# yinwoods/k8s-scheduler

Measured on AMD Instinct MI355X. Metric: pod-node evaluations/sec, higher is better.
Workload: dtype f64

## Files before the change

k8s-scheduler_amd/csrc/ksched_pipe.hip:

```cpp
#include <hip/hip_fp16.h>
#include <hip/hip_runtime.h>

#include <cstdio>
#include <cstdlib>

#include "ksched_commit.h"
#include "ksched_merge.h"

#ifndef KSCHED_PIPE_PART
#define KSCHED_PIPE_PART 0
#endif

namespace ksched {

namespace {

constexpr int kSW = kPipeScoreWaves;
constexpr int kMT = kPipeMergeThreads;
constexpr int kMW = kMT / 64;
constexpr int kMS = kPipeMergeSlots;
constexpr int kPU = 4;
#ifndef KSCHED_XCHG_DEBUG
#define KSCHED_XCHG_DEBUG 0
#endif
constexpr int kSPU = 4;
constexpr int kPairCap = 48;
constexpr int kPairMax = 1024;

__device__ __forceinline__ int bperm(int v, int src) { return __builtin_amdgcn_ds_bpermute(src << 2, v); }
__device__ __forceinline__ int64_t bperm64(int64_t v, int src) {
    const uint32_t lo = (uint32_t)bperm((int)(uint32_t)(uint64_t)v, src);
    const uint32_t hi = (uint32_t)bperm((int)(uint32_t)((uint64_t)v >> 32), src);
    return (int64_t)(((uint64_t)hi << 32) | lo);
}
__device__ __forceinline__ int wave_incl_sum(int v) {
    const int lane = (int)__lane_id();
#pragma unroll
    for (int d = 1; d < 64; d <<= 1) {
        const int t = bperm(v, lane >= d ? lane - d : 0);
        v += lane >= d ? t : 0;
    }
    return v;
}

__device__ __forceinline__ void role_sync(unsigned *ctr, unsigned &target, unsigned nwaves) {
    __builtin_amdgcn_fence(__ATOMIC_RELEASE, "workgroup");
    target += nwaves;
    if ((threadIdx.x & 63) == 0) __hip_atomic_fetch_add(ctr, 1u, __ATOMIC_RELAXED, __HIP_MEMORY_SCOPE_WORKGROUP);
    while (__hip_atomic_load(ctr, __ATOMIC_RELAXED, __HIP_MEMORY_SCOPE_WORKGROUP) < target) __builtin_amdgcn_s_sleep(1);
    __builtin_amdgcn_fence(__ATOMIC_ACQUIRE, "workgroup");
}

struct alignas(16) PipeCtl {
    unsigned sbar, mbar;
    int32_t s_stop, m_stop;
    int64_t s_p0, s_done;
    int64_t m_p0, m_done;
    int32_t c_stop;
    int32_t s_ex;
    int32_t s_scr;
    int32_t s_pairs;
    int32_t n_ok, n_err;
    int64_t n_p0, n_done;
};
constexpr size_t kPipeCtlBytes = 128;
static_assert(sizeof(PipeCtl) <= kPipeCtlBytes, "PipeCtl");

__device__ __forceinline__ bool spin_ge(const PersistArgs &P, int slot, const unsigned long long *p,
                                        unsigned long long v, unsigned long long *seen) {
    return poll_ge(p, v, P.timeout_ticks, &P.ctl->polls_rmw, seen, P.prog ? P.prog + kProgWords * slot + 2 : nullptr);
}

__device__ __forceinline__ void set_err(int32_t *err, int32_t code) { atomicCAS(err, 0, code); }

__device__ __forceinline__ void st_sys(uint64_t *p, uint64_t v) {
    __hip_atomic_store(p, v, __ATOMIC_RELAXED, __HIP_MEMORY_SCOPE_SYSTEM);
}
__device__ __forceinline__ uint64_t ld_sys(const uint64_t *p) {
    return __hip_atomic_load(p, __ATOMIC_RELAXED, __HIP_MEMORY_SCOPE_SYSTEM);
}
__device__ __forceinline__ bool granule_wait(const uint64_t *p, uint32_t tag, int64_t limit, uint32_t *word) {
    const uint32_t t16 = gran_tag(tag);
    if (!gran_dec(ld_sys(p), t16, word)) {
        const uint64_t t0 = wall_clock64();
        do {
            if ((int64_t)(wall_clock64() - t0) > limit) return false;
            __builtin_amdgcn_s_sleep(1);
        } while (!gran_dec(ld_sys(p), t16, word));
    }
    return true;
}

template <int K>
__device__ __forceinline__ void rank_merge_msgs(const uint32_t *all, int R, Rec *out, int64_t *out_fc) {
    constexpr int MW = msg_words(K);
    const int lane = threadIdx.x & 63;
    const bool has = lane < R;
    const uint32_t *msg = all + (has ? lane : 0) * MW;
    auto rec_key = [&](int q) {
        return __longlong_as_double((long long)(((uint64_t)msg[q * kRecWords + 1] << 32) | msg[q * kRecWords]));
    };
    int n = 0;
    if (has) {
#pragma unroll
        for (int q = 0; q < K; ++q) n += msg[q * kRecWords + 3] != 0;
    }
    const bool cut = has && msg[13] != 0;
    int64_t cnt = has ? (int64_t)(((uint64_t)msg[K * kRecWords + 1] << 32) | msg[K * kRecWords]) : 0;
    cnt = wave_sum_i64(cnt);
    double ck = (cut && n > 0) ? rec_key(n - 1) : -__builtin_inf();
    int32_t ci = (cut && n > 0) ? (int32_t)msg[(n - 1) * kRecWords + 2] : kNoIdx;
    const bool anycut = __ballot(cut) != 0;
    {
        int32_t aux = 0;
        wave_argbest(ck, ci, aux);
    }
    int h = 0;
    double mk = -__builtin_inf();
    int32_t mi = kNoIdx, msrc = -1;
    for (int r = 0; r < K; ++r) {
        double k = (h < n) ? rec_key(h) : -__builtin_inf();
        int32_t ix = (h < n) ? (int32_t)msg[h * kRecWords + 2] : kNoIdx;
        int32_t src = lane * K + h;
        wave_argbest(k, ix, src);
        if (ix == kNoIdx) break;
        if (src == lane * K + h) ++h;
        if (lane == r) { mk = k; mi = ix; msrc = src; }
// ... 52 lines not shown
#pragma unroll
        for (int j = i; j >= 1; --j) {
            const uint32_t a = t[j - 1], c = t[j];
            t[j - 1] = a > c ? a : c;
            t[j] = a > c ? c : a;
        }
    }
}

template <int KC>
__device__ __forceinline__ void topk_merge_u32(uint32_t (&t)[KC], const uint32_t (&u)[KC]) {
    uint32_t v[KC];
#pragma unroll
    for (int q = 0; q < KC; ++q) v[q] = t[q] > u[KC - 1 - q] ? t[q] : u[KC - 1 - q];
#pragma unroll
    for (int d = KC / 2; d >= 1; d >>= 1) {
#pragma unroll
        for (int i = 0; i < KC; ++i) {
            if ((i & d) == 0) {
                const uint32_t a = v[i], b = v[i + d];
                v[i] = a > b ? a : b;
                v[i + d] = a > b ? b : a;
            }
        }
    }
#pragma unroll
    for (int q = 0; q < KC; ++q) t[q] = v[q];
}

template <int S, int KC>
__device__ __forceinline__ void fold_stage(double (&k)[KC], int32_t (&ix)[KC]) {
    double ok[KC];
    int32_t oi[KC];
#pragma unroll
    for (int q = 0; q < KC; ++q) {
        ok[q] = wpartner_f64<S>(k[q]);
        oi[q] = (int32_t)wpartner<S>((uint32_t)ix[q]);
    }
    double vk[KC];
    int32_t vi[KC];
#pragma unroll
    for (int q = 0; q < KC; ++q) {
        const bool t = better(ok[KC - 1 - q], oi[KC - 1 - q], k[q], ix[q]);
        vk[q] = t ? ok[KC - 1 - q] : k[q];
        vi[q] = t ? oi[KC - 1 - q] : ix[q];
    }
#pragma unroll
    for (int d = KC / 2; d >= 1; d >>= 1) {
#pragma unroll
        for (int i = 0; i < KC; ++i) {
            if ((i & d) == 0) {
                const bool t = better(vk[i + d], vi[i + d], vk[i], vi[i]);
                const double a = vk[i], bb = vk[i + d];
                const int32_t ai = vi[i], bi = vi[i + d];
                vk[i] = t ? bb : a; vi[i] = t ? bi : ai;
                vk[i + d] = t ? a : bb; vi[i + d] = t ? ai : bi;
            }
        }
    }
#pragma unroll
    for (int q = 0; q < KC; ++q) { k[q] = vk[q]; ix[q] = vi[q]; }
}

template <int KC, int K>
struct ScoreLayout {
    static constexpr size_t fold_list_bytes = (size_t)kSW * KC * 64 * 12 + 64 * 4;
    __host__ __device__ static size_t fold_bytes(int R) {
        const size_t scr = (size_t)kSW * KC * 64 * 4 + kSW * 4 + (size_t)2 * kSW * ((R + kSW - 1) / kSW) * 2;
        return scr > fold_list_bytes ? scr : fold_list_bytes;
    }
    __host__ __device__ static size_t rows_off() { return kPipeCtlBytes; }
    __host__ __device__ static size_t fold_off(int R) { return kPipeCtlBytes + (size_t)R * sizeof(NodeRec); }
    __host__ __device__ static size_t total(int R) { return fold_off(R) + (fold_bytes(R) + 15) / 16 * 16; }
    __host__ __device__ static size_t ysq_off(int R) { return total(R); }
    __host__ __device__ static size_t total_screen(int R) { return total(R) + (size_t)R * 16; }
    __host__ __device__ static size_t hrec_off(int R) { return total_screen(R); }
    __host__ __device__ static int hrec_qw(int R) { return ((R + kSW - 1) / kSW + 1) / 2 * 2; }
    __host__ __device__ static size_t hrec_bytes(int R) { return (size_t)kSW * hrec_qw(R) * 64 * 2; }
    __host__ __device__ static size_t total_with_hrec(int R) { return total_screen(R) + hrec_bytes(R); }
    __host__ __device__ static size_t pair_off(int R) {
        const size_t QW = (size_t)(R + kSW - 1) / kSW;
        return ((size_t)kSW * KC * 64 * 4 + kSW * 4 + 4 * kSW * QW + 15) / 16 * 16;
    }
    static constexpr size_t pair_bytes = 64 * 4 * 2 + (size_t)kPairMax * 8 + (size_t)64 * kPairCap * 2;
    __host__ __device__ static bool pairs_fit(int R) { return pair_off(R) + pair_bytes <= (size_t)kSW * KC * 64 * 12; }
};
struct PairArea {
    uint32_t *cnt;
    uint32_t *nel;
    double *key;
    uint16_t *row;
};

struct alignas(16) MergeCtl {
    unsigned mbar;
    int32_t m_stop;
    int64_t m_p0, m_done;
    int32_t m_w, pad;
    unsigned long long m_q;
};
template <int KC, int K>
struct MergeLayout {
    static constexpr size_t ctl_bytes = 64;
    static constexpr size_t merge_bytes = (sizeof(MergeSmem<KC, K, kMT>) + 15) / 16 * 16;
    static constexpr size_t msg_bytes = ((size_t)(1 + kMaxXchgRanks) * msg_words(K) * 4 + 15) / 16 * 16;
    static constexpr size_t slot_bytes = ctl_bytes + merge_bytes + msg_bytes;
    static constexpr size_t total = kMS * slot_bytes;
};
static_assert(sizeof(MergeCtl) <= 64, "MergeCtl");

constexpr size_t kCanaryBytes = 128;
constexpr size_t commit_loc_bytes() { return (sizeof(PersistLocal) + 15) / 16 * 16 + kCanaryBytes; }
template <int K>
constexpr size_t commit_total_bytes() { return commit_loc_bytes() + spc_lds_bytes<K, kPipeThreads, true>(); }
static_assert(commit_total_bytes<16>() <= 160 * 1024, "the persistent commit's LDS (lag-3 slots)");
static_assert(commit_loc_bytes() + spc_small_bytes<16, kPipeThreads, true>() + 256 <= 65536,
              "the persistent commit's arrays in front of S reach LDS immediate offsets");

template <int KC, int K, int PRIO, int DOM, bool LAB, bool F53>
__device__ __forceinline__ void score_role(const PersistArgs &P, char *smem, const int g) {
    PipeCtl *pc = reinterpret_cast<PipeCtl *>(smem);
    const int R = P.rows_per_wg;
    NodeRec *rows = reinterpret_cast<NodeRec *>(smem + ScoreLayout<KC, K>::rows_off());
    char *fold = smem + ScoreLayout<KC, K>::fold_off(R);
    float4 *ysq = reinterpret_cast<float4 *>(smem + ScoreLayout<KC, K>::ysq_off(R));
    uint16_t *hrec = reinterpret_cast<uint16_t *>(smem + ScoreLayout<KC, K>::hrec_off(R));
    int32_t *s_cnt = reinterpret_cast<int32_t *>(fold + (size_t)kSW * KC * 64 * 12);
    PairArea pr;
    {
        char *pa = fold + ScoreLayout<KC, K>::pair_off(R);
        pr.cnt = reinterpret_cast<uint32_t *>(pa);
        pr.nel = pr.cnt + 64;
        pr.key = reinterpret_cast<double *>(pa + 512);
        pr.row = reinterpret_cast<uint16_t *>(pa + 512 + (size_t)kPairMax * 8);
    }
    constexpr int kST = kSW * 64;
    const int tid = threadIdx.x;
    const int lane = tid & 63;
    const int wave = __builtin_amdgcn_readfirstlane(tid >> 6);
    const int G = P.G;
    const int64_t n = P.n_local, NP = P.pods.p;
    Ctl *ctl = P.ctl;
    auto sync = [&]() { __syncthreads(); };
    for (int e = tid; e < R * 6; e += kST) {
        const int r = e / 6, piece = e % 6;
        const int64_t j = g + (int64_t)r * G;
        if (j < n) reinterpret_cast<int4 *>(rows + r)[piece] = reinterpret_cast<const int4 *>(P.nodes + j)[piece];
    }
    if (tid == 0) pc->n_ok = 0;
    sync();
    if (P.screen_ok) {
        for (int r = tid; r < R; r += kST) {
            const NodeRec &nd = rows[r];
            ysq[r] = make_float4(screen_recip(nd.a[0]), screen_recip(nd.a[1]), screen_recip(nd.a[2]), 0.0f);
        }
    }
    const double y3 = recip(3.0);
    constexpr bool kScreen = PRIO == kPrioResource && F53;
    constexpr bool kPairs = kScreen;
    const bool pairs_ok = kPairs && !P.no_pairs && ScoreLayout<KC, K>::pairs_fit(R);
    constexpr int kScreenOffBatches = 16;
    constexpr bool kPrefetch = kSW > 8;
    int64_t scr_off_until = 0;
    int64_t ex_rows = 0, scan_rows = 0;
    const int64_t Rvalid = (n - g + G - 1) / G;
    int64_t nact = 0;
    int idle = 0;
    unsigned long long early_c = 0;
    unsigned long long pre_c = 0;
    auto load_apply = [&](int64_t bb, int stop, int64_t *p0v, int64_t *donev, int *errv) {
        int nxv = 0;
        u32x4 x0 = {0u, 0u, 0u, 0u}, x1 = {0u, 0u, 0u, 0u}, x2 = {0u, 0u, 0u, 0u};
        const XBuf *xb =
            reinterpret_cast<const XBuf *>(P.xring + (size_t)((bb >= kPipeLag ? bb - kPipeLag : 0) % 4) * P.xbuf_bytes);
        if (lane == 0) {
            *p0v = (int64_t)ld_coh(&ctl->plan[bb % kPlanRing]);
            *donev = bb >= kPipeLag ? (int64_t)ld_coh(&ctl->cursor_at[(bb - kPipeLag) % kPlanRing]) : 0;
            *errv = __hip_atomic_load(P.err, __ATOMIC_RELAXED, __HIP_MEMORY_SCOPE_AGENT);
        }
        if (bb >= kPipeLag && !stop) {
            const uint64_t hdr = ld_coh(&xb->count);
            nxv = (uint32_t)(hdr >> 32) == (uint32_t)(bb - kPipeLag) ? (int)(uint32_t)hdr : 0;
            if (lane < 2 * P.B) {
                const __amdgpu_buffer_rsrc_t rs = coh_rsrc(xb->e);
                const uint32_t o = (uint32_t)lane * kXRecPipe;
                x0 = ld_coh16(rs, o); x1 = ld_coh16(rs, o + 16); x2 = ld_coh16(rs, o + 32);
            }
        }
        auto apply = [&](const u32x4 &c0, const u32x4 &c1, const u32x4 &c2) {
            const int64_t j = (int64_t)(int32_t)c0.y - P.node_offset;
            if (j < 0 || j >= n || j % G != g) return;
            const int64_t a0 = w64(c0.z, c0.w), a1 = w64(c1.y, c1.z), a2 = w64(c1.w, c2.y);
            set_row(rows + j / G, a0, a1, a2);
            if (P.screen_ok) ysq[j / G] = make_float4(screen_recip(a0), screen_recip(a1), screen_recip(a2), 0.0f);
            st_coh(&P.nodes[j].a[0], (uint64_t)a0);
            st_coh(&P.nodes[j].a[1], (uint64_t)a1);
            st_coh(&P.nodes[j].a[2], (uint64_t)a2);
        };
        if (lane < nxv) apply(x0, x1, x2);
        for (int e = 64 + lane; e < nxv; e += 64) {
            const __amdgpu_buffer_rsrc_t rs = coh_rsrc(xb->e);
            const uint32_t o = (uint32_t)e * kXRecPipe;
            apply(ld_coh16(rs, o), ld_coh16(rs, o + 16), ld_coh16(rs, o + 32));
        }
    };
    for (int64_t b = 0;; ++b) {
        if (wave == 0) {
            if (kPrefetch && __builtin_amdgcn_readfirstlane(pc->n_ok)) {
                if (lane == 0) {
                    pc->s_p0 = pc->n_p0;
                    pc->s_done = pc->n_done;
                    pc->s_stop = pc->n_err != 0 ? 3 : 0;
                    pc->s_scr = kScreen && P.screen_ok && !P.no_screen && b >= scr_off_until;
                    pc->s_ex = 0;
                    pc->n_ok = 0;
                }
            } else {
                int stop = 0;
                jitter_at(P.jitter, b, 1);
                if (lane == 0) {
                    unsigned long long seen = 0;
                    const unsigned long long need = (unsigned long long)(b - kPipeLag + 1);
                    if (b >= kPipeLag && early_c < need) {
                        prog_at(P, g, b, kProgWaitCommit, 0);
                        if (!spin_ge(P, g, &ctl->committed_x[g % kCtlReplicas].v, need, &seen)) {
                            set_err(P.err, kErrWaitCommit);
                            prog_at(P, g, b, kProgWaitCommit | kProgTimedOut, seen);
                            stop = 2;
                        }
                    }
                    if (g == 0) trace_at(P, b, 6);
                }
                stop = __builtin_amdgcn_readfirstlane(stop);
                int64_t p0v = 0, donev = 0;
                int errv = 0;
                load_apply(b, stop, &p0v, &donev, &errv);
                if (lane == 0) {
                    pc->s_p0 = p0v;
                    pc->s_done = donev;
                    pc->s_stop = errv != 0 ? 3 : stop;
                    pc->s_scr = kScreen && P.screen_ok && !P.no_screen && b >= scr_off_until;
                    pc->s_ex = 0;
                }
            }
        }
        sync();
        if (kPrefetch && wave == kSW - 1) asm volatile("s_waitcnt vmcnt(0)" ::: "memory");
        if (pc->s_stop) return;
        const int64_t p0 = pc->s_p0;
        if (pc->s_done >= NP) break;
        if (p0 < 0 || p0 >= NP) {
            if (tid == 0) prog_at(P, g, b, kProgIdle, (uint64_t)p0);
            if (++idle > kPlanRing) {
                if (tid == 0) set_err(P.err, kErrScorePlan);
                return;
            }
            sync();
            continue;
        }
        idle = 0;
        ++nact;
        if (tid == 0) {
            if (g == 0) trace_at(P, b, 0);
            prog_at(P, g, b, kProgScan, 0);
        }
        const uint64_t t_go = ((P.trace || P.trace_wg) && tid == 0) ? wall_clock64() : 0;
        if (tid < 64) s_cnt[tid] = 0;
        if (kPairs && tid < 64) { pr.cnt[tid] = 0; pr.nel[tid] = 0; }
        bool pairs = false;
        int pT = 0, pincl = 0, pexcl = 0;
        const int64_t pod = p0 + lane;
        const bool active = (lane < P.B) && (pod < NP);
        const int64_t rc = active ? P.pods.rc[pod] : 0;
        const int64_t rm = active ? P.pods.rm[pod] : 0;
        const int64_t rp = active ? P.pods.rp[pod] : 0;
        const uint64_t sel = (LAB && active) ? P.pods.sel[pod] : 0;
        const double rcf = (double)rc, rmf = (double)rm, rpf = (double)rp;
        double key[KC];
        int32_t idx[KC];
#pragma unroll
        for (int q = 0; q < KC; ++q) { key[q] = -__builtin_inf(); idx[q] = kNoIdx; }
        int32_t cnt = 0;
        const bool scr = kScreen && pc->s_scr;
        if (scr) {
            const float qc = screen_req(rc), qm = screen_req(rm), qp = screen_req(rp);
            const int Rv = (int)((n - g + G - 1) / G);
            const int QW = (R + kSW - 1) / kSW;
            const bool keep_h = P.screen_h != 0;
            uint32_t *hw = reinterpret_cast<uint32_t *>(hrec) + (size_t)wave * (ScoreLayout<KC, K>::hrec_qw(R) / 2) * 64 + lane;
            auto row_screen = [&](int r, const float4 &y, bool valid, bool *f, bool *el, bool *lo_ok) {
                const float c = qc * y.x, m = qm * y.y, p = qp * y.z;
                bool okc = c < kFracLo, okm = m < kFracLo, okp = p < kFracLo;
                const bool amb = !(okc || c > kFracHi) || !(okm || m > kFracHi) || !(okp || p > kFracHi);
                uint64_t lab = 0;
                if (__ballot(valid && amb)) {
                    const NodeRec &nd = rows[r];
                    okc = nd.a[0] >= rc; okm = nd.a[1] >= rm; okp = nd.a[2] >= rp;
                }
                if (LAB) lab = rows[r].labels;
                *f = okc & okm & okp & (!LAB || (lab & sel) == sel);
                *el = DOM == kDomAll || *f;
                return screen_q(c, m, p, okc, okm, okp, lo_ok);
            };
            uint32_t t[KC];
#pragma unroll
            for (int q = 0; q < KC; ++q) t[q] = 0u;
            uint32_t *sl = reinterpret_cast<uint32_t *>(fold);
            int32_t *qcnt = reinterpret_cast<int32_t *>(sl + kSW * KC * 64);
            uint16_t *qrow = reinterpret_cast<uint16_t *>(qcnt + kSW);
            uint16_t *arow = qrow + kSW * QW;
            int na = 0;
            if (keep_h) {
                static_assert(kSPU % 2 == 0, "pass 1 stores the records of row pairs");
                for (int r0 = wave; r0 < Rv; r0 += kSW * kSPU) {
                    float4 yv[kSPU];
                    uint64_t lb[kSPU];
#pragma unroll
                    for (int u = 0; u < kSPU; ++u) {
                        const int r = r0 + u * kSW;
                        yv[u] = ysq[r < Rv ? r : r0];
                        lb[u] = LAB ? rows[r < Rv ? r : r0].labels : 0ull;
                    }
                    uint32_t xs[kSPU];
                    uint32_t hh[kSPU];
                    uint32_t ambm = 0;
                    float ww[kSPU];
                    uint32_t nrm[kSPU];
#pragma unroll
                    for (int u = 0; u < kSPU; ++u) {
                        const int r = r0 + u * kSW;
                        const bool valid = r < Rv;
                        const ScreenV sv = screen_fast(qc * yv[u].x, qm * yv[u].y, qp * yv[u].z);
                        const float v = sv.v;
                        const bool amb = sv.amb, rf = sv.rf;
                        const bool f = rf && (!LAB || (lb[u] & sel) == sel);
                        const bool el = DOM == kDomAll || f;
                        const bool lo_ok = !(rf && sv.mx >= 0.999f) && v > kScreenEps;
                        cnt += (valid && f && !amb) ? 1 : 0;
                        xs[u] = (valid && active && el && lo_ok && !amb) ? __float_as_uint(v + (1.0f - kScreenEps)) : 0u;
                        ww[u] = __builtin_fmaxf((rf ? 10.0f : kNfBase) - v, 0.0f);
                        nrm[u] = (!amb && el) ? (rf ? 1u : 0x8001u) : 0u;
                        hh[u] = amb ? 0u : 0xffffu;
                        ambm |= (valid && amb) ? 1u << u : 0u;
                    }
#pragma unroll
                    for (int u = 0; u < kSPU; u += 2) {
                        const uint32_t rec = __builtin_bit_cast(uint32_t, __builtin_amdgcn_cvt_pkrtz(ww[u], ww[u + 1]));
                        const uint32_t w2 = (nrm[u] ? ((rec & 0xffffu) | (nrm[u] & 0x8000u)) : hh[u]) |
                                            ((nrm[u + 1] ? ((rec >> 16) | (nrm[u + 1] & 0x8000u)) : hh[u + 1]) << 16);
                        if (r0 + u * kSW < Rv) hw[(size_t)(((r0 - wave) / kSW + u) / 2) * 64] = w2;
                    }
                    if (__ballot(ambm != 0)) {
#pragma unroll
                        for (int u = 0; u < kSPU; ++u) {
                            const bool anya = __ballot((ambm >> u) & 1u) != 0;
                            if (lane == 0 && na < QW) arow[wave * QW + na] = (uint16_t)(r0 + u * kSW);
                            na += anya ? 1 : 0;
                        }
                    }
                    bound_slots<KC>(t, xs);
                }
                for (int e = 0; e < na; ++e) {
                    const int r = arow[wave * QW + e];
                    const NodeRec &nd = rows[r];
                    const float4 y = ysq[r];
                    const float c = qc * y.x, m = qm * y.y, p = qp * y.z;
                    const bool amb = !(c < kFracLo || c > kFracHi) || !(m < kFracLo || m > kFracHi) ||
                                     !(p < kFracLo || p > kFracHi);
                    cnt += (amb && fits(rc, rm, rp, sel, nd.a[0], nd.a[1], nd.a[2], nd.labels, LAB)) ? 1 : 0;
                }
            } else {
                for (int r0 = wave; r0 < Rv; r0 += kSW * kSPU) {
                    float4 yv[kSPU];
#pragma unroll
                    for (int u = 0; u < kSPU; ++u) {
                        const int r = r0 + u * kSW;
                        yv[u] = ysq[r < Rv ? r : r0];
                    }
                    uint32_t xs[kSPU];
#pragma unroll
                    for (int u = 0; u < kSPU; ++u) {
                        const int r = r0 + u * kSW;
                        const bool valid = r < Rv;
                        bool f, el, lo_ok;
                        const float v = row_screen(valid ? r : r0, yv[u], valid, &f, &el, &lo_ok);
                        cnt += (valid && f) ? 1 : 0;
                        xs[u] = (valid && active && el && lo_ok) ? __float_as_uint(v + (1.0f - kScreenEps)) : 0u;
                    }
                    bound_slots<KC>(t, xs);
                }
            }
            if (g == 0 && tid == 0) trace_at(P, b, 11);
            sort_desc_u32<KC>(t);
#pragma unroll
            for (int q = 0; q < KC; ++q) sl[(wave * KC + q) * 64 + lane] = t[q];
            sync();
            for (int w = 1; w < kSW; ++w) {
                const int ow = (wave + w) % kSW;
                uint32_t u[KC];
#pragma unroll
                for (int q = 0; q < KC; ++q) u[q] = sl[(ow * KC + q) * 64 + lane];
                topk_merge_u32<KC>(t, u);
            }
            const float L = __uint_as_float(t[KC - 1]);
            if (g == 0 && tid == 0) trace_at(P, b, 12);
            if (cnt) atomicAdd(&s_cnt[lane], cnt);
            int qn = 0;
            auto add_pair = [&](bool need, int r) {
                if (kPairs && need) {
                    const uint32_t s = atomicAdd(&pr.cnt[lane], 1u);
                    if (s < (uint32_t)kPairCap) pr.row[lane * kPairCap + s] = (uint16_t)r;
                }
            };
            if (keep_h) {
                const int nr = (Rv - wave + kSW - 1) / kSW;
                const int tq = active ? screen_rec_threshold(L) : -1;
                const int tqn = active ? screen_rec_threshold_nf(L) : -1;
                for (int i0 = 0; i0 < nr; i0 += 8) {
                    uint16_t hv[8];
#pragma unroll
                    for (int u = 0; u < 8; u += 2) {
                        const uint32_t x = hw[(size_t)((i0 + u < nr ? i0 + u : i0) / 2) * 64];
                        hv[u] = (uint16_t)x;
                        hv[u + 1] = (uint16_t)(x >> 16);
                    }
                    uint32_t grp = 0;
                    uint32_t mine = 0;
#pragma unroll
                    for (int u = 0; u < 8; ++u) {
                        const bool nd = screen_rec_needed(hv[u], tq, tqn);
                        const uint64_t bm = __builtin_amdgcn_ballot_w64(nd);
                        grp |= (bm != 0 ? 1u : 0u) << u;
                        mine |= (nd ? 1u : 0u) << u;
                    }
                    if (nr - i0 < 8) grp &= (1u << (nr - i0)) - 1u;
                    if (lane < 8 && ((grp >> lane) & 1u))
                        qrow[wave * QW + qn + __builtin_popcount(grp & ((1u << lane) - 1u))] =
                            (uint16_t)(wave + (i0 + lane) * kSW);
                    qn += __builtin_popcount(grp);
                    if (kPairs && grp) {
                        uint32_t mm = mine & grp;
                        const int c = __builtin_popcount(mm);
                        uint32_t s = c ? atomicAdd(&pr.cnt[lane], (uint32_t)c) : 0u;
                        for (; mm; mm &= mm - 1u, ++s)
                            if (s < (uint32_t)kPairCap)
                                pr.row[lane * kPairCap + s] = (uint16_t)(wave + (i0 + __builtin_ctz(mm)) * kSW);
                    }
                }
            } else {
                for (int r0 = wave; r0 < Rv; r0 += kSW * kSPU) {
                    float4 yv[kSPU];
#pragma unroll
                    for (int u = 0; u < kSPU; ++u) {
                        const int r = r0 + u * kSW;
                        yv[u] = ysq[r < Rv ? r : r0];
                    }
#pragma unroll
                    for (int u = 0; u < kSPU; ++u) {
                        const int r = r0 + u * kSW;
                        const bool valid = r < Rv;
                        bool f, el, lo_ok;
                        const float v = row_screen(valid ? r : r0, yv[u], valid, &f, &el, &lo_ok);
                        const bool need = valid && active && el && !(v + (1.0f + kScreenEps) < L);
                        const bool any = __ballot(need) != 0;
                        if (lane == 0 && qn < QW) qrow[wave * QW + qn] = (uint16_t)r;
                        qn += any ? 1 : 0;
                        if (any) add_pair(need, r);
                    }
                }
            }
            if (lane == 0) qcnt[wave] = qn;
            if (g == 0 && tid == 0) trace_at(P, b, 14);
            sync();
            int base[kSW], tot = 0;
#pragma unroll
            for (int w = 0; w < kSW; ++w) { base[w] = tot; tot += qcnt[w]; }
            if (kPairs) {
                const int c = (int)pr.cnt[lane];
                pincl = wave_incl_sum(c);
                pexcl = pincl - c;
                pT = __builtin_amdgcn_readlane(pincl, 63);
                pairs = pairs_ok && __ballot(c > kPairCap) == 0 && pT <= kPairMax;
            }
            if (pairs) {
                for (int e0 = wave * 64; e0 < pT; e0 += kST) {
                    const int e = e0 + lane;
                    const int ec = e < pT ? e : pT - 1;
                    int p = 0;
#pragma unroll
                    for (int st = 32; st; st >>= 1) p += bperm(pincl, p + st - 1) <= ec ? st : 0;
                    const int s = ec - bperm(pexcl, p);
                    const int64_t qc = bperm64(rc, p), qm = bperm64(rm, p), qp = bperm64(rp, p);
                    const uint64_t qs = LAB ? (uint64_t)bperm64((int64_t)sel, p) : 0ull;
                    if (e < pT) {
                        const int r = pr.row[p * kPairCap + s];
                        const NodeRec &nd = rows[r];
                        const int64_t ac = nd.a[0], am = nd.a[1], ap = nd.a[2];
                        const bool f = fits(qc, qm, qp, qs, ac, am, ap, nd.labels, LAB);
                        double k;
                        const bool el = pair_key_fast<PRIO, DOM, F53>(f, qc, qm, qp, (double)qc, (double)qm, (double)qp, ac,
                                                                      am, ap, nd.af[0], nd.af[1], nd.af[2], nd.y[0],
                                                                      nd.y[1], nd.y[2], y3, nd.price, &k);
                        pr.key[e] = el ? k : -__builtin_inf();
                        if (el) atomicAdd(&pr.nel[p], 1u);
                    }
                }
            } else
            for (int e = wave; e < tot; e += kSW) {
                int w = 0;
#pragma unroll
                for (int v = 1; v < kSW; ++v) w += e >= base[v] ? 1 : 0;
                const int r = qrow[w * QW + (e - base[w])];
                const NodeRec &nd = rows[r];
                const int64_t ac = nd.a[0], am = nd.a[1], ap = nd.a[2];
                const bool f = fits(rc, rm, rp, sel, ac, am, ap, nd.labels, LAB);
                double k;
                const bool el = pair_key_fast<PRIO, DOM, F53>(f, rc, rm, rp, rcf, rmf, rpf, ac, am, ap, nd.af[0], nd.af[1],
                                                              nd.af[2], nd.y[0], nd.y[1], nd.y[2], y3, nd.price, &k);
                if (el) list_insert_ordered<KC>(key, idx, k, (int32_t)(P.node_offset + g + (int64_t)r * G));
            }
            if (wave == 0 && lane == 0) { pc->s_ex = tot; pc->s_pairs = pairs ? pT : -1; }
        } else
        for (int r0 = wave; r0 < R; r0 += kSW * kPU) {
            double ks[kPU];
#pragma unroll
            for (int u = 0; u < kPU; ++u) {
                const int r = r0 + u * kSW;
                const int64_t j = g + (int64_t)r * G;
                ks[u] = -__builtin_inf();
                if (r < R && j < n) {
                    const NodeRec &nd = rows[r];
                    const int64_t ac = nd.a[0], am = nd.a[1], ap = nd.a[2];
                    const bool f = fits(rc, rm, rp, sel, ac, am, ap, nd.labels, LAB);
                    cnt += f;
                    double k;
                    const bool el = pair_key_fast<PRIO, DOM, F53>(f, rc, rm, rp, rcf, rmf, rpf, ac, am, ap, nd.af[0],
                                                                  nd.af[1], nd.af[2], nd.y[0], nd.y[1], nd.y[2], y3,
                                                                  nd.price, &k);
                    ks[u] = el ? k : -__builtin_inf();
                }
            }
#pragma unroll
            for (int u = 0; u < kPU; ++u) {
                double ck = ks[u];
                int32_t ci = (int32_t)(P.node_offset + g + (int64_t)(r0 + u * kSW) * G);
                bool moved = false;
#pragma unroll
                for (int q = 0; q < KC; ++q) {
                    const bool sw = moved || ck > key[q];
                    moved = sw;
                    const double tk = key[q];
                    const int32_t ti = idx[q];
                    key[q] = sw ? ck : tk; idx[q] = sw ? ci : ti;
                    ck = sw ? tk : ck; ci = sw ? ti : ci;
                }
            }
        }
        if (g == 0 && tid == 0) trace_at(P, b, 8);
        const uint64_t t_scan = (P.trace && tid == 0) ? wall_clock64() : 0;
        if (tid == 0) early_c = __hip_atomic_load(&ctl->committed_x[g % kCtlReplicas].v, __ATOMIC_RELAXED,
                                                  __HIP_MEMORY_SCOPE_AGENT);
        if (kPrefetch && wave == kSW - 1 && lane == 0)
            pre_c = __hip_atomic_load(&ctl->committed_x[g % kCtlReplicas].v, __ATOMIC_RELAXED, __HIP_MEMORY_SCOPE_AGENT);
        sync();
        if (g == 0 && tid == 0) trace_at(P, b, 9);
        auto prefetch_next = [&]() {
            const unsigned long long need = (unsigned long long)(b + 1 - kPipeLag + 1);
            int ok = 0;
            if (lane == 0) {
                ok = b + 1 < kPipeLag || pre_c >= need;
                if (!ok) ok = __hip_atomic_load(&ctl->committed_x[g % kCtlReplicas].v, __ATOMIC_RELAXED,
                                                __HIP_MEMORY_SCOPE_AGENT) >= need;
            }
            ok = __builtin_amdgcn_readfirstlane(ok);
            if (ok) {
                if (g == 0 && lane == 0) trace_at(P, b + 1, 6);
                int64_t p0v = 0, donev = 0;
                int errv = 0;
                load_apply(b + 1, 0, &p0v, &donev, &errv);
                if (lane == 0) { pc->n_p0 = p0v; pc->n_done = donev; pc->n_err = errv; }
            }
            if (lane == 0) pc->n_ok = ok;
        };
        const size_t part_elems = (size_t)P.B * G;
        Cand *part = P.part + (size_t)(b % kPipeLag) * part_elems * KC;
        auto store_entry = [&](int pl, int q, double kk, int32_t ii) {
            const uint64_t kb = (uint64_t)__double_as_longlong(kk);
            const uint32_t tag = (uint32_t)((b + 1) & 0xffff) << 16;
            const u32x4 v = {(uint32_t)kb, (uint32_t)(kb >> 32), (uint32_t)ii, tag | (q == 0 ? (uint32_t)s_cnt[pl] : 0u)};
            st_coh16(coh_rsrc(part), (uint32_t)((((size_t)pl * G + g) * KC + q) * sizeof(Cand)), v);
        };
        if (pairs) {
            if (kPrefetch && wave == kSW - 1) {
                prefetch_next();
            } else {
                constexpr int RW = kPrefetch ? kSW - 1 : kSW;
                for (int e0 = wave * 64; e0 < pT; e0 += RW * 64) {
                    const int e = e0 + lane;
                    const int ec = e < pT ? e : pT - 1;
                    int p = 0;
#pragma unroll
                    for (int st = 32; st; st >>= 1) p += bperm(pincl, p + st - 1) <= ec ? st : 0;
                    const int ex = bperm(pexcl, p), in = bperm(pincl, p);
                    if (e < pT) {
                        const double k = pr.key[e];
                        if (k != -__builtin_inf()) {
                            const uint16_t *prow = pr.row + p * kPairCap;
                            const int r = prow[e - ex];
                            int rank = 0;
                            int e2 = ex;
                            for (; e2 + 4 <= in; e2 += 4) {
                                double k2[4];
                                int r2[4];
#pragma unroll
                                for (int u = 0; u < 4; ++u) { k2[u] = pr.key[e2 + u]; r2[u] = prow[e2 + u - ex]; }
#pragma unroll
                                for (int u = 0; u < 4; ++u) rank += (k2[u] > k || (k2[u] == k && r2[u] < r)) ? 1 : 0;
                            }
                            for (; e2 < in; ++e2) {
                                const double k2 = pr.key[e2];
                                const int r2 = prow[e2 - ex];
                                rank += (k2 > k || (k2 == k && r2 < r)) ? 1 : 0;
                            }
                            if (rank < KC && p < P.B && p0 + p < NP)
                                store_entry(p, rank, k, (int32_t)(P.node_offset + g + (int64_t)r * G));
                        }
                    }
                }
                if (wave == 0 && lane < P.B && p0 + lane < NP) {
                    for (int q = (int)pr.nel[lane]; q < KC; ++q) store_entry(lane, q, -__builtin_inf(), kNoIdx);
                }
            }
            if (g == 0 && tid == 0) trace_at(P, b, 10);
            if (wave == 0) asm volatile("s_waitcnt vmcnt(0)" ::: "memory");
        } else {
        if (!scr && cnt) atomicAdd(&s_cnt[lane], cnt);
        double *fk = reinterpret_cast<double *>(fold);
        int32_t *fi = reinterpret_cast<int32_t *>(fold + (size_t)kSW * KC * 64 * 8);
#pragma unroll
        for (int q = 0; q < KC; ++q) {
            fk[(wave * KC + q) * 64 + lane] = key[q];
            fi[(wave * KC + q) * 64 + lane] = idx[q];
        }
        sync();
        static_assert(kSW >= 8 && kSW <= 16, "the fold deals 8 pods to each of the first 8 waves");
        const int pl = wave * 8 + (lane >> 3);
        const int src = lane & 7;
        const bool folds = wave < 8;
        if (kPrefetch && wave == kSW - 1) prefetch_next();
        if (folds) {
#pragma unroll
            for (int q = 0; q < KC; ++q) {
                key[q] = fk[(src * KC + q) * 64 + pl];
                idx[q] = fi[(src * KC + q) * 64 + pl];
            }
            if (src + 8 < kSW) {
#pragma unroll
                for (int q = 0; q < KC; ++q) {
                    const int32_t oi = fi[((src + 8) * KC + q) * 64 + pl];
                    if (oi == kNoIdx) break;
                    list_insert_ordered<KC>(key, idx, fk[((src + 8) * KC + q) * 64 + pl], oi);
                }
            }
            fold_stage<0, KC>(key, idx);
            fold_stage<1, KC>(key, idx);
            fold_stage<2, KC>(key, idx);
        }
        if (g == 0 && tid == 0) trace_at(P, b, 10);
        if (wave == 0) asm volatile("s_waitcnt vmcnt(0)" ::: "memory");
        if (folds && pl < P.B && p0 + pl < NP && src < KC) {
            double kk = key[0];
            int32_t ii = idx[0];
#pragma unroll
            for (int q = 1; q < KC; ++q) {
                kk = src == q ? key[q] : kk;
                ii = src == q ? idx[q] : ii;
            }
            store_entry(pl, src, kk, ii);
        }
        }
        sync();
        if (wave == 0) {
            if (scr && 2 * pc->s_ex > R) scr_off_until = b + 1 + kScreenOffBatches;
            if (scr && g == 0 && lane == 0 && P.trace && b < P.trace_cap)
                P.trace[b * kTraceCols + 13] = (uint64_t)(uint32_t)pc->s_ex | (uint64_t)(uint32_t)pc->s_pairs << 32;
            if (lane == 0) { ex_rows += scr ? pc->s_ex : Rvalid; scan_rows += Rvalid; }
            jitter_at(P.jitter, b, 2);
            const int slot = (int)((nact - 1) % 4);
            if (lane == 0) {
                if (g == 0) trace_at(P, b, 5);
                const unsigned long long old = __hip_atomic_fetch_add(&ctl->arrive[slot].v, 1ull, __ATOMIC_RELAXED,
                                                                      __HIP_MEMORY_SCOPE_AGENT);
                const unsigned long long use = (unsigned long long)((nact - 1) / 4);
                if (old + 1 == (use + 1) * (unsigned long long)G) trace_at(P, b, 1);
                prog_at(P, g, b, kProgArrived, old + 1);
                if (P.trace) prog_add(P, g, t_scan - t_go, wall_clock64() - t_go);
                if (P.trace_wg && b < P.trace_cap)
                    P.trace_wg[b * G + g] = (t_go & 0xffffffffull) | (wall_clock64() << 32);
            }
        }
    }
    if (tid == 0 && P.prog) { P.prog[kProgWords * g + 4] = (uint64_t)ex_rows; P.prog[kProgWords * g + 5] = (uint64_t)scan_rows; }
    for (int e = tid; e < R * 6; e += kST) {
        const int r = e / 6, piece = e % 6;
        const int64_t j = g + (int64_t)r * G;
        if (j < n) reinterpret_cast<int4 *>(P.nodes + j)[piece] = reinterpret_cast<const int4 *>(rows + r)[piece];
    }
}

// ... 451 lines not shown
        ca.batch = b;
        ca.cursor_at = &ctl->cursor_at[b % kPlanRing];
        ca.dbg = P.cdbg;
        ca.trace_row = (P.trace && b < P.trace_cap) ? P.trace + b * kTraceCols : nullptr;
        ca.loc = &loc;
        ca.rescue = P.rescue;
        ca.xp = &P;
        ca.dbg_act = nact - 1;
        ca.rescue_n = P.B;
        ca.rescue_max = P.rescue_max;
        ca.rescue_rate = P.rescue_rate;
        ca.rescue_look = P.rescue_look;
        ca.rescue_cap = P.rescue_cap;
        ca.rescue_low = P.rescue_low;
        ca.touch_screen = P.touch_screen;
        ca.inh = P.inh;
        ca.timeout_ticks = P.timeout_ticks;
        ca.err = P.err;
        const int rc = commit_spc_batch<K, PRIO, DOM, LAB, F53, true, kPipeThreads>(ca, cs, &pre, wait_merged, handoff);
        if (rc == 2) return;
        if (rc == 0) {
            if (threadIdx.x == 0) atomicCAS(P.err, 0, kErrWaitMerged);
            if (threadIdx.x < 64) publish_committed_all(ctl, 1ull << 62);
            return;
        }
        __syncthreads();
        if (threadIdx.x < kCanaryBytes / 4 && canary[threadIdx.x] != (0xA5A5A5A5u ^ threadIdx.x)) {
            if (atomicCAS(P.err, 0, kErrLdsCanary) == 0 && P.prog)
                P.prog[kProgWords * cslot + 2] = (uint64_t)b << 32 | (uint64_t)threadIdx.x << 16 | (canary[threadIdx.x] & 0xffffu);
        }
        if (threadIdx.x == 0) {
            trace_at(P, b, 4);
            prog_at(P, cslot, b, kProgCommitted, 0);
        }
        if (loc.cursor >= P.pods.p) {
            if (threadIdx.x < 64) publish_committed_all(ctl, 1ull << 62);
            return;
        }
    }
}

template <int KC, int K, int PRIO, int DOM, bool LAB, bool F53>
__global__ __launch_bounds__(kPipeThreads) void k_pipe(PipeLaunch L) {
    extern __shared__ __attribute__((aligned(16))) char smem[];
    int r = 0;
#pragma unroll
    for (int i = 1; i < kMaxLocalRanks; ++i) r += (i < L.R && (int)blockIdx.x >= L.base[i]) ? 1 : 0;
    const PersistArgs &P = L.P[r];
    const int blk = (int)blockIdx.x - L.base[r];
    if (P.poison_lds) {
        const int role = blk < kCommitWGs ? 1 : (blk < kCommitWGs + P.G ? 2 : 4);
        const uint32_t fill = (P.lds_fill_role & 8) ? P.lds_fill ^ ((uint32_t)role * 0x01010101u) : P.lds_fill;
        if (P.lds_fill_role & role)
            for (int i = (int)threadIdx.x; i < P.poison_lds / 4; i += kPipeThreads)
                if (4 * i >= P.lds_fill_lo && 4 * i < P.lds_fill_hi) reinterpret_cast<uint32_t *>(smem)[i] = fill;
        __syncthreads();
    }
    if (blk < kCommitWGs) {
        commit_role<K, PRIO, DOM, LAB, F53>(P, smem, blk);
        return;
    }
    if (blk < kCommitWGs + P.G) {
        PipeCtl *pc = reinterpret_cast<PipeCtl *>(smem);
        if (threadIdx.x == 0) { pc->sbar = 0; pc->mbar = 0; }
        __syncthreads();
        score_role<KC, K, PRIO, DOM, LAB, F53>(P, smem, blk - kCommitWGs);
        return;
    }
    const int slot = (int)threadIdx.x / kMT;
    const int id = (blk - kCommitWGs - P.G) * kMS + slot;
    char *sbase = smem + (size_t)slot * MergeLayout<KC, K>::slot_bytes;
    if (threadIdx.x % kMT == 0) reinterpret_cast<MergeCtl *>(sbase)->mbar = 0;
    __syncthreads();
    if (id < P.B) merge_role<KC, K, PRIO, DOM, LAB, F53>(P, sbase, id);
}

template <int KC, int K, int PRIO, int DOM, bool LAB, bool F53>
hipError_t pipe_one(const PipeLaunch &L0, int launch, PipeInfo *info, hipStream_t s) {
    auto fn = k_pipe<KC, K, PRIO, DOM, LAB, F53>;
    PipeLaunch L = L0;
    constexpr size_t kLds = (size_t)160 * 1024;
    int R = 0;
    for (int r = 0; r < L.R; ++r) R = L.P[r].rows_per_wg > R ? L.P[r].rows_per_wg : R;
    const int sh = ScoreLayout<KC, K>::total_with_hrec(R) <= kLds ? 1 : 0;
    const int so = ScoreLayout<KC, K>::total_screen(R) <= kLds ? 1 : 0;
    for (int r = 0; r < L.R; ++r) { L.P[r].screen_h = sh; L.P[r].screen_ok = so; }
    const size_t sl = sh ? ScoreLayout<KC, K>::total_with_hrec(R)
                         : (so ? ScoreLayout<KC, K>::total_screen(R) : ScoreLayout<KC, K>::total(R));
    const size_t cl = commit_total_bytes<K>(), ml = MergeLayout<KC, K>::total;
    const size_t lds = sl > cl ? (sl > ml ? sl : ml) : (cl > ml ? cl : ml);
    if (info) {
        hipFuncAttributes at{};
        hipError_t e = hipFuncGetAttributes(&at, (const void *)fn);
        if (e != hipSuccess) return e;
        info->lds = lds;
        info->static_lds = at.sharedSizeBytes;
        info->vgprs = at.numRegs;
        info->spill = at.localSizeBytes;
        info->occ = 0;
        if (lds + at.sharedSizeBytes <= kLds) {
            e = hipFuncSetAttribute((const void *)fn, hipFuncAttributeMaxDynamicSharedMemorySize, (int)lds);
            if (e == hipSuccess) e = hipOccupancyMaxActiveBlocksPerMultiprocessor(&info->occ, fn, kPipeThreads, lds);
            if (e != hipSuccess) return e;
        }
    }
    if (!launch) return hipSuccess;
    if (L.R < 1 || L.R > kMaxLocalRanks || L.base[0] != 0) return hipErrorInvalidValue;
    for (int r = 0; r < L.R; ++r) {
        const PersistArgs &a = L.P[r];
        if (a.G > kMT || a.B > 64 || a.M * kMS < a.B || L.base[r + 1] - L.base[r] != kCommitWGs + a.G + a.M ||
            a.rows_per_wg >= 65536)
            return hipErrorInvalidValue;
    }
    hipError_t e = hipFuncSetAttribute((const void *)fn, hipFuncAttributeMaxDynamicSharedMemorySize, (int)lds);
    if (e != hipSuccess) return e;
    if (launch == 2) {
        hipLaunchKernelGGL(fn, dim3(L.base[L.R]), dim3(kPipeThreads), lds, s, L);
        return hipGetLastError();
    }
    void *args[] = {&L};
    return hipLaunchCooperativeKernel((const void *)fn, dim3(L.base[L.R]), dim3(kPipeThreads), args, (unsigned)lds, s);
}

template <int PRIO, int DOM, bool LAB, bool F53>
hipError_t pipe_kk(int KC, int K, const PipeLaunch &a, int launch, PipeInfo *info, hipStream_t s) {
    if (KC == 4 && K == 4) return pipe_one<4, 4, PRIO, DOM, LAB, F53>(a, launch, info, s);
    if (KC == 4 && K == 8) return pipe_one<4, 8, PRIO, DOM, LAB, F53>(a, launch, info, s);
    if (KC == 4 && K == 16) return pipe_one<4, 16, PRIO, DOM, LAB, F53>(a, launch, info, s);
    if (KC == 8 && K == 8) return pipe_one<8, 8, PRIO, DOM, LAB, F53>(a, launch, info, s);
    if (KC == 8 && K == 16) return pipe_one<8, 16, PRIO, DOM, LAB, F53>(a, launch, info, s);
    return hipErrorNotSupported;
}

template <int PRIO, int DOM>
hipError_t pipe_lf(int KC, int K, bool lab, bool f53, const PipeLaunch &a, int launch, PipeInfo *info, hipStream_t s) {
    if (PRIO == kPrioPrice) f53 = false;
    if (lab) return f53 ? pipe_kk<PRIO, DOM, true, true>(KC, K, a, launch, info, s)
                        : pipe_kk<PRIO, DOM, true, false>(KC, K, a, launch, info, s);
    return f53 ? pipe_kk<PRIO, DOM, false, true>(KC, K, a, launch, info, s)
               : pipe_kk<PRIO, DOM, false, false>(KC, K, a, launch, info, s);
}

}

#if KSCHED_PIPE_PART == 0
hipError_t pipe_part_price(int KC, int K, bool lab, bool f53, const PipeLaunch &a, int launch, PipeInfo *info,
                           hipStream_t s) {
    return pipe_lf<kPrioPrice, kDomFeasible>(KC, K, lab, f53, a, launch, info, s);
}

__global__ __launch_bounds__(64) void k_xchg_min(PersistArgs P, int32_t mine, int32_t *out) {
    const int lane = threadIdx.x;
    const size_t off = (size_t)4 * P.R * P.B * (size_t)P.xchg_stride;
    const uint32_t tag = P.epoch0;
    if (lane < P.R) st_sys(reinterpret_cast<uint64_t *>(P.rx_peer[lane] + off) + P.rank, gran_enc((uint32_t)mine, gran_tag(tag)));
    int32_t v = 0x7fffffff;
    bool ok = true;
    if (lane < P.R) {
        uint32_t w = 0;
        ok = granule_wait(reinterpret_cast<const uint64_t *>(P.rx_peer[P.rank] + off) + lane, tag, P.timeout_ticks, &w);
        v = (int32_t)w;
    }
    v = wave_min_i32(v);
    const bool bad = __ballot(!ok) != 0;
    if (lane == 0) {
        if (bad) set_err(P.err, kErrRankBarrier);
        *out = bad ? -1 : v;
// ... 22 lines not shown
```

Baseline: 269.4 billion.

## Replace per-wave candidate lists with 64-bit row bitmasks in screened scoring

For small KC, each lane builds a 64-bit mask of rows needing exact evaluation from the half-precision screen records. Lanes OR-reduce the masks across the wave so the fallback path compacts rows from the mask, and the pair pass carries its per-lane pair state into the ranking pass instead of recomputing the binary search and reloading key and row. This aims to cut LDS traffic and bpermute searches, at the cost of extra LDS for the wave masks. It also restricts the hrec path to at most 64 rows per wave.

```diff
diff --git a/k8s-scheduler_amd/csrc/ksched_pipe.hip b/k8s-scheduler_amd/csrc/ksched_pipe.hip
--- a/k8s-scheduler_amd/csrc/ksched_pipe.hip
+++ b/k8s-scheduler_amd/csrc/ksched_pipe.hip
@@ -42,7 +42,15 @@
     }
     return v;
 }
-
+template <int S>
+__device__ __forceinline__ uint64_t or_stage(uint64_t v) {
+    return v | (((uint64_t)wpartner<S>((uint32_t)(v >> 32)) << 32) | wpartner<S>((uint32_t)v));
+}
+__device__ __forceinline__ uint64_t wave_or_u64(uint64_t v) {
+    v = or_stage<0>(v); v = or_stage<1>(v); v = or_stage<2>(v);
+    v = or_stage<3>(v); v = or_stage<4>(v); v = or_stage<5>(v);
+    return v;
+}
 __device__ __forceinline__ void role_sync(unsigned *ctr, unsigned &target, unsigned nwaves) {
     __builtin_amdgcn_fence(__ATOMIC_RELEASE, "workgroup");
     target += nwaves;
@@ -261,7 +269,7 @@
         const size_t QW = (size_t)(R + kSW - 1) / kSW;
         return ((size_t)kSW * KC * 64 * 4 + kSW * 4 + 4 * kSW * QW + 15) / 16 * 16;
     }
-    static constexpr size_t pair_bytes = 64 * 4 * 2 + (size_t)kPairMax * 8 + (size_t)64 * kPairCap * 2;
+    static constexpr size_t pair_bytes = 64 * 4 * 2 + (size_t)kPairMax * 8 + (size_t)64 * kPairCap * 2 + kSW * 8;
     __host__ __device__ static bool pairs_fit(int R) { return pair_off(R) + pair_bytes <= (size_t)kSW * KC * 64 * 12; }
 };
 struct PairArea {
@@ -269,6 +277,7 @@
     uint32_t *nel;
     double *key;
     uint16_t *row;
+    uint64_t *wmask;
 };
 
 struct alignas(16) MergeCtl {
@@ -312,6 +321,7 @@
         pr.nel = pr.cnt + 64;
         pr.key = reinterpret_cast<double *>(pa + 512);
         pr.row = reinterpret_cast<uint16_t *>(pa + 512 + (size_t)kPairMax * 8);
+        pr.wmask = reinterpret_cast<uint64_t *>(pa + 512 + (size_t)kPairMax * 8 + (size_t)64 * kPairCap * 2);
     }
     constexpr int kST = kSW * 64;
     const int tid = threadIdx.x;
@@ -337,6 +347,7 @@
     const double y3 = recip(3.0);
     constexpr bool kScreen = PRIO == kPrioResource && F53;
     constexpr bool kPairs = kScreen;
+    constexpr bool kMasks = KC <= 4;
     const bool pairs_ok = kPairs && !P.no_pairs && ScoreLayout<KC, K>::pairs_fit(R);
     constexpr int kScreenOffBatches = 16;
     constexpr bool kPrefetch = kSW > 8;
@@ -448,6 +459,8 @@
         if (kPairs && tid < 64) { pr.cnt[tid] = 0; pr.nel[tid] = 0; }
         bool pairs = false;
         int pT = 0, pincl = 0, pexcl = 0;
+        int hp = 0, hex = 0, hin = 0, hr = 0;
+        double hk = -__builtin_inf();
         const int64_t pod = p0 + lane;
         const bool active = (lane < P.B) && (pod < NP);
         const int64_t rc = active ? P.pods.rc[pod] : 0;
@@ -466,6 +479,7 @@
             const int Rv = (int)((n - g + G - 1) / G);
             const int QW = (R + kSW - 1) / kSW;
             const bool keep_h = P.screen_h != 0;
+            const bool masks = keep_h && kMasks;
             uint32_t *hw = reinterpret_cast<uint32_t *>(hrec) + (size_t)wave * (ScoreLayout<KC, K>::hrec_qw(R) / 2) * 64 + lane;
             auto row_screen = [&](int r, const float4 &y, bool valid, bool *f, bool *el, bool *lo_ok) {
                 const float c = qc * y.x, m = qm * y.y, p = qp * y.z;
@@ -595,6 +609,29 @@
                 const int nr = (Rv - wave + kSW - 1) / kSW;
                 const int tq = active ? screen_rec_threshold(L) : -1;
                 const int tqn = active ? screen_rec_threshold_nf(L) : -1;
+                if constexpr (kMasks) {
+                uint64_t mine = 0;
+                for (int i0 = 0; i0 < nr; i0 += 16) {
+                    uint32_t x[8];
+#pragma unroll
+                    for (int u = 0; u < 8; ++u) x[u] = hw[(size_t)((i0 + 2 * u < nr ? i0 + 2 * u : i0) / 2) * 64];
+                    uint32_t m16 = 0;
+#pragma unroll
+                    for (int u = 0; u < 8; ++u) {
+                        m16 |= (screen_rec_needed(x[u] & 0xffffu, tq, tqn) ? 1u : 0u) << (2 * u);
+                        m16 |= (screen_rec_needed(x[u] >> 16, tq, tqn) ? 1u : 0u) << (2 * u + 1);
+                    }
+                    mine |= (uint64_t)m16 << i0;
+                }
+                if (nr < 64) mine &= (1ull << nr) - 1ull;
+                const int c = __builtin_popcountll(mine);
+                uint32_t s = c ? atomicAdd(&pr.cnt[lane], (uint32_t)c) : 0u;
+                for (uint64_t mm = mine; mm; mm &= mm - 1ull, ++s)
+                    if (s < (uint32_t)kPairCap)
+                        pr.row[lane * kPairCap + s] = (uint16_t)(wave + __builtin_ctzll(mm) * kSW);
+                const uint64_t wm = wave_or_u64(mine);
+                if (lane == 0) pr.wmask[wave] = wm;
+                } else {
                 for (int i0 = 0; i0 < nr; i0 += 8) {
                     uint16_t hv[8];
 #pragma unroll
@@ -626,6 +663,7 @@
                                 pr.row[lane * kPairCap + s] = (uint16_t)(wave + (i0 + __builtin_ctz(mm)) * kSW);
                     }
                 }
+                }
             } else {
                 for (int r0 = wave; r0 < Rv; r0 += kSW * kSPU) {
                     float4 yv[kSPU];
@@ -648,12 +686,9 @@
                     }
                 }
             }
-            if (lane == 0) qcnt[wave] = qn;
+            if (!masks && lane == 0) qcnt[wave] = qn;
             if (g == 0 && tid == 0) trace_at(P, b, 14);
             sync();
-            int base[kSW], tot = 0;
-#pragma unroll
-            for (int w = 0; w < kSW; ++w) { base[w] = tot; tot += qcnt[w]; }
             if (kPairs) {
                 const int c = (int)pr.cnt[lane];
                 pincl = wave_incl_sum(c);
@@ -661,6 +696,12 @@
                 pT = __builtin_amdgcn_readlane(pincl, 63);
                 pairs = pairs_ok && __ballot(c > kPairCap) == 0 && pT <= kPairMax;
             }
+            constexpr int kStatWave = kSW - 2;
+            int base[kSW], tot = 0;
+            if (!masks) {
+#pragma unroll
+                for (int w = 0; w < kSW; ++w) { base[w] = tot; tot += qcnt[w]; }
+            }
             if (pairs) {
                 for (int e0 = wave * 64; e0 < pT; e0 += kST) {
                     const int e = e0 + lane;
@@ -668,11 +709,12 @@
                     int p = 0;
 #pragma unroll
                     for (int st = 32; st; st >>= 1) p += bperm(pincl, p + st - 1) <= ec ? st : 0;
-                    const int s = ec - bperm(pexcl, p);
+                    const int ex = bperm(pexcl, p);
+                    const int in = kMasks ? bperm(pincl, p) : 0;
                     const int64_t qc = bperm64(rc, p), qm = bperm64(rm, p), qp = bperm64(rp, p);
                     const uint64_t qs = LAB ? (uint64_t)bperm64((int64_t)sel, p) : 0ull;
                     if (e < pT) {
-                        const int r = pr.row[p * kPairCap + s];
+                        const int r = pr.row[p * kPairCap + (ec - ex)];
                         const NodeRec &nd = rows[r];
                         const int64_t ac = nd.a[0], am = nd.a[1], ap = nd.a[2];
                         const bool f = fits(qc, qm, qp, qs, ac, am, ap, nd.labels, LAB);
@@ -682,9 +724,21 @@
                                                                       nd.y[1], nd.y[2], y3, nd.price, &k);
                         pr.key[e] = el ? k : -__builtin_inf();
                         if (el) atomicAdd(&pr.nel[p], 1u);
-                    }
-                }
-            } else
+                        if constexpr (kMasks) { hp = p; hex = ex; hin = in; hr = r; hk = el ? k : -__builtin_inf(); }
+                    }
+                }
+                if (masks && wave == kStatWave)
+                    tot = (int)wave_sum_i64(lane < kSW ? (int64_t)__builtin_popcountll(pr.wmask[lane]) : 0);
+            } else {
+            if (masks) {
+                const uint64_t wm = pr.wmask[wave];
+                if ((wm >> lane) & 1ull)
+                    qrow[wave * QW + __builtin_popcountll(wm & ((1ull << lane) - 1ull))] = (uint16_t)(wave + lane * kSW);
+                if (lane == 0) qcnt[wave] = __builtin_popcountll(wm);
+                sync();
+#pragma unroll
+                for (int w = 0; w < kSW; ++w) { base[w] = tot; tot += qcnt[w]; }
+            }
             for (int e = wave; e < tot; e += kSW) {
                 int w = 0;
 #pragma unroll
@@ -698,7 +752,8 @@
                                                               nd.af[2], nd.y[0], nd.y[1], nd.y[2], y3, nd.price, &k);
                 if (el) list_insert_ordered<KC>(key, idx, k, (int32_t)(P.node_offset + g + (int64_t)r * G));
             }
-            if (wave == 0 && lane == 0) { pc->s_ex = tot; pc->s_pairs = pairs ? pT : -1; }
+            }
+            if (wave == (masks ? kStatWave : 0) && lane == 0) { pc->s_ex = tot; pc->s_pairs = pairs ? pT : -1; }
         } else
         for (int r0 = wave; r0 < R; r0 += kSW * kPU) {
             double ks[kPU];
@@ -774,36 +829,39 @@
                 prefetch_next();
             } else {
                 constexpr int RW = kPrefetch ? kSW - 1 : kSW;
+                const bool held = kMasks && pT <= RW * 64;
                 for (int e0 = wave * 64; e0 < pT; e0 += RW * 64) {
                     const int e = e0 + lane;
-                    const int ec = e < pT ? e : pT - 1;
-                    int p = 0;
-#pragma unroll
-                    for (int st = 32; st; st >>= 1) p += bperm(pincl, p + st - 1) <= ec ? st : 0;
-                    const int ex = bperm(pexcl, p), in = bperm(pincl, p);
-                    if (e < pT) {
-                        const double k = pr.key[e];
-                        if (k != -__builtin_inf()) {
-                            const uint16_t *prow = pr.row + p * kPairCap;
-                            const int r = prow[e - ex];
-                            int rank = 0;
-                            int e2 = ex;
-                            for (; e2 + 4 <= in; e2 += 4) {
-                                double k2[4];
-                                int r2[4];
-#pragma unroll
-                                for (int u = 0; u < 4; ++u) { k2[u] = pr.key[e2 + u]; r2[u] = prow[e2 + u - ex]; }
-#pragma unroll
-                                for (int u = 0; u < 4; ++u) rank += (k2[u] > k || (k2[u] == k && r2[u] < r)) ? 1 : 0;
-                            }
-                            for (; e2 < in; ++e2) {
-                                const double k2 = pr.key[e2];
-                                const int r2 = prow[e2 - ex];
-                                rank += (k2 > k || (k2 == k && r2 < r)) ? 1 : 0;
-                            }
-                            if (rank < KC && p < P.B && p0 + p < NP)
-                                store_entry(p, rank, k, (int32_t)(P.node_offset + g + (int64_t)r * G));
+                    int p = hp, ex = hex, in = hin, r = hr;
+                    double k = hk;
+                    if (!held) {
+                        const int ec = e < pT ? e : pT - 1;
+                        p = 0;
+#pragma unroll
+                        for (int st = 32; st; st >>= 1) p += bperm(pincl, p + st - 1) <= ec ? st : 0;
+                        ex = bperm(pexcl, p);
+                        in = bperm(pincl, p);
+                        if (e < pT) { k = pr.key[e]; r = pr.row[p * kPairCap + e - ex]; }
+                    }
+                    if (e < pT && k != -__builtin_inf()) {
+                        const uint16_t *prow = pr.row + p * kPairCap;
+                        int rank = 0;
+                        int e2 = ex;
+                        for (; e2 + 4 <= in; e2 += 4) {
+                            double k2[4];
+                            int r2[4];
+#pragma unroll
+                            for (int u = 0; u < 4; ++u) { k2[u] = pr.key[e2 + u]; r2[u] = prow[e2 + u - ex]; }
+#pragma unroll
+                            for (int u = 0; u < 4; ++u) rank += (k2[u] > k || (k2[u] == k && r2[u] < r)) ? 1 : 0;
                         }
+                        for (; e2 < in; ++e2) {
+                            const double k2 = pr.key[e2];
+                            const int r2 = prow[e2 - ex];
+                            rank += (k2 > k || (k2 == k && r2 < r)) ? 1 : 0;
+                        }
+                        if (rank < KC && p < P.B && p0 + p < NP)
+                            store_entry(p, rank, k, (int32_t)(P.node_offset + g + (int64_t)r * G));
                     }
                 }
                 if (wave == 0 && lane < P.B && p0 + lane < NP) {
@@ -1421,7 +1479,7 @@
     constexpr size_t kLds = (size_t)160 * 1024;
     int R = 0;
     for (int r = 0; r < L.R; ++r) R = L.P[r].rows_per_wg > R ? L.P[r].rows_per_wg : R;
-    const int sh = ScoreLayout<KC, K>::total_with_hrec(R) <= kLds ? 1 : 0;
+    const int sh = ScoreLayout<KC, K>::total_with_hrec(R) <= kLds && ScoreLayout<KC, K>::hrec_qw(R) <= 64 ? 1 : 0;
     const int so = ScoreLayout<KC, K>::total_screen(R) <= kLds ? 1 : 0;
     for (int r = 0; r < L.R; ++r) { L.P[r].screen_h = sh; L.P[r].screen_ok = so; }
     const size_t sl = sh ? ScoreLayout<KC, K>::total_with_hrec(R)
```

Result: faster. 279.3 billion (median of 6 runs) (+3.7%).
